# klukaszek/MRI-RayTracer

Hardware: AMD Instinct MI355X
Metric: live Msamples/s, 512^3 fp32 volume @ 1024^2 x 512 steps (gradient shading + ERT) (higher is better)
Workload: dtype f32

## Files before the change

include/mrirt.h:

```cpp
#ifndef MRIRT_H
#define MRIRT_H

#include <stdint.h>

#ifdef __cplusplus
extern "C" {
#endif

#define MRIRT_ABI_VERSION 4

typedef enum MrirtStatus {
    MRIRT_OK = 0,
    MRIRT_ERR_NULL = -1,
    MRIRT_ERR_DIMS = -2,
    MRIRT_ERR_LAYOUT = -3,
    MRIRT_ERR_LAUNCH = -4,
    MRIRT_ERR_ARG = -5,
    MRIRT_ERR_NO_DEVICE = -6
} MrirtStatus;


typedef struct MrirtBratsParams {
    uint32_t imageSize[2]; float fovY; float pad0;
    float eye[3]; float pad1;
// ... 135 lines not shown
int mrirt_build_macro_labels(const uint32_t* labels_linear, const uint32_t dims[3], uint32_t* macro_any, void* stream);
int mrirt_render_brats_skip(const MrirtBratsParams* params, const MrirtRenderExt* ext,
                            const void* const vol[4], const void* labels, const void* preds,
                            const MrirtSkip* skip, void* out_rgba, int64_t pitch_px,
                            uint64_t* stats_dev, void* stream);
int mrirt_brats_skip_applicable(const MrirtBratsParams* params, const MrirtRenderExt* ext, const void* const vol[4],
                                const void* labels, const void* preds, const MrirtSkip* skip);
typedef enum MrirtKernelFamily {
    MRIRT_KERNEL_NONE = 0, MRIRT_KERNEL_GENERIC = 1, MRIRT_KERNEL_PIPELINED = 2, MRIRT_KERNEL_ROLLING = 3,
    MRIRT_KERNEL_SLAB = 4, MRIRT_KERNEL_RING = 5,
    MRIRT_KERNEL_SKIPPING = 16, MRIRT_KERNEL_LABEL_CELLS = 32
} MrirtKernelFamily;
int mrirt_brats_kernel_family(const MrirtBratsParams* params, const MrirtRenderExt* ext, const void* const vol[4],
                              const void* labels, const void* preds, const MrirtSkip* skip);

int64_t mrirt_tiles_for_rank(uint32_t width, uint32_t height, uint32_t tileSize, uint32_t rank, uint32_t world);
int mrirt_detile(const void* gathered, void* frame, uint32_t width, uint32_t height, int64_t pitch_px,
                 uint32_t tileSize, uint32_t world, uint32_t tileSkew, uint32_t outFormat, void* stream);

typedef enum MrirtInrKind {
    MRIRT_INR_FOURIER_RELU = 0,
    MRIRT_INR_SIREN = 1,
    MRIRT_INR_RAW_RELU = 2,
    MRIRT_INR_RAW_SIREN = 3
} MrirtInrKind;

typedef struct MrirtInrDesc {
    uint32_t kind;
    uint32_t numLayers;
    uint32_t inDim;
// ... 184 lines not shown
```

mri-raytracer_amd/_lib.py:

```python
from __future__ import annotations

import ctypes as C
import os
import pathlib
import subprocess
import sys
from typing import List, Optional

PKG_DIR = pathlib.Path(__file__).resolve().parent
CSRC = PKG_DIR / "csrc"
INCLUDE = PKG_DIR.parent / "include"
SO_PATH = pathlib.Path(os.environ.get("MRIRT_LIB", PKG_DIR / "libmrirt.so"))
HIP_SOURCES = ["brats_march.hip", "brats_skip.hip", "brats_c5.hip", "brats_slab.hip", "brats_ring.hip", "brats_backward.hip", "brats_soft.hip", "volume_march.hip", "grid_ops.hip", "inr_mlp.hip",
               "inr_stream.hip", "inr_ws.hip", "inr_refine.hip", "inr_train.hip", "inr_optim.hip", "inr_muon.hip", "inr_lossx.hip", "mesh_rt.hip", "edt.hip", "surface.hip", "abort_trace.cpp"]
HIPCC_FLAGS = ["-O3", "--offload-arch=gfx950", "-ffp-contract=off", "-fPIC", "-shared", "-std=c++17", "-Wall"]

ABI_SYMBOLS = [
    "mrirt_render_brats", "mrirt_render_brats_ex", "mrirt_brats_sample_counts", "mrirt_brats_emit_samples",
    "mrirt_render_brats_stream", "mrirt_brats_inr_scratch_bytes", "mrirt_render_brats_inr", "mrirt_brick_elems", "mrirt_brick_grid",
    "mrirt_unbrick_grid", "mrirt_vec4_elems", "mrirt_vga_elems", "mrirt_build_vec4_grid", "mrirt_build_label_cells", "mrirt_build_mod4_grid", "mrirt_bc4_decode", "mrirt_macro_cells", "mrirt_skip_mask_words",
    "mrirt_build_macro_max", "mrirt_build_macro_labels", "mrirt_render_brats_skip", "mrirt_render_volume", "mrirt_build_cell8", "mrirt_render_sdf", "mrirt_render_mesh", "mrirt_tiles_for_rank",
    "mrirt_detile", "mrirt_inr_pack_bytes", "mrirt_inr_pack_weights", "mrirt_inr_calibrate", "mrirt_inr_forward", "mrirt_inr_forward_refined",
    "mrirt_inr_predict_volume", "mrirt_abi_version", "mrirt_status_string", "mrirt_last_hip_error",
    "mrirt_sizeof", "mrirt_brats_skip_applicable", "mrirt_brats_kernel_family", "mrirt_install_abort_trace",
    "mrirt_edt_scratch_bytes", "mrirt_edt_squared", "mrirt_hausdorff",
    "mrirt_surface_scratch_bytes", "mrirt_surface_count", "mrirt_surface_extract",
    "mrirt_render_brats_backward", "mrirt_render_brats_soft", "mrirt_render_brats_soft_backward",
    "mrirt_inr_train_scratch_bytes", "mrirt_inr_loss_scratch_bytes", "mrirt_inr_forward_f32", "mrirt_inr_loss", "mrirt_inr_backward",
    "mrirt_inr_sample_batch", "mrirt_inr_adamw_scratch_bytes", "mrirt_inr_adamw_step", "mrirt_inr_lr_schedule",
    "mrirt_inr_train_run_scratch_bytes", "mrirt_inr_train_run",
    "mrirt_siren_train_scratch_bytes", "mrirt_siren_forward_f32", "mrirt_siren_backward",
    "mrirt_siren_train_run_scratch_bytes", "mrirt_siren_train_run",
    "mrirt_muon_scratch_bytes", "mrirt_muon_orthogonalize", "mrirt_muon_step",
    "mrirt_inr_train_run_muon_scratch_bytes", "mrirt_inr_train_run_muon",
    "mrirt_inr_loss_ext_scratch_bytes", "mrirt_inr_loss_ext", "mrirt_inr_tumour_count", "mrirt_inr_tumour_index_scratch_bytes",
    "mrirt_inr_tumour_index", "mrirt_inr_sample_batch_mix", "mrirt_inr_train_run_ext_scratch_bytes", "mrirt_inr_train_run_ext",
]

ABI_VERSION = 4
OK = 0
LAYOUT_LINEAR, LAYOUT_BRICK, LAYOUT_VG, LAYOUT_QUAD, LAYOUT_VGA, LAYOUT_LABCELL, LAYOUT_MOD4 = 0, 1, 2, 3, 4, 5, 6
MATH_STRICT, MATH_FAST = 0, 1
OUT_RGBA32F, OUT_RGBA16F = 0, 1
VOX_U32X4, VOX_U8, VOX_F32, VOX_CELL8 = 0, 1, 2, 3
INR_FOURIER_RELU, INR_SIREN = 0, 1
INR_NO_WEIGHT_STATIONARY, INR_NO_REFINE, INR_MARK_ONLY = 1, 2, 4
KERNEL_NONE, KERNEL_GENERIC, KERNEL_PIPELINED, KERNEL_ROLLING, KERNEL_SLAB, KERNEL_RING = 0, 1, 2, 3, 4, 5
KERNEL_SKIPPING, KERNEL_LABEL_CELLS = 16, 32

f32, u32 = C.c_float, C.c_uint32

# ... 89 lines not shown
                ("edemaFpWeight", f32), ("tverskyAlpha", f32), ("tverskyBeta", f32), ("tverskyWeight", f32), ("edemaLogitReg", f32),
                ("edemaClass", u32), ("flags", u32)]


class InrTumourIndex(C.Structure):
    _fields_ = [("index", C.c_void_p), ("offsets", C.c_void_p)]


class InrTrainExt(C.Structure):
    _fields_ = [("loss", C.POINTER(InrLossExt)), ("muon", C.POINTER(Muon)), ("tumour", InrTumourIndex), ("nTumour", C.c_int64)]


class Skip(C.Structure):
    _fields_ = [("macroUb", C.c_void_p * 4), ("macroSeg", C.c_void_p), ("macroPred", C.c_void_p), ("mask", C.c_void_p),
                ("maskWords", u32), ("mapReady", u32)]


class MrirtError(RuntimeError):
    def __init__(self, status: int, where: str):
        l = lib()
        msg = l.mrirt_status_string(status).decode()
        extra = f" (hipError {l.mrirt_last_hip_error()})" if status == -4 else ""
        super().__init__(f"{where}: {msg}{extra} [status {status}]")
        self.status = status


OBJ_DIR = PKG_DIR / "build"
MAX_BUILD_JOBS = 16


# ... 131 lines not shown
    l.mrirt_build_mod4_grid.restype = i32
    l.mrirt_macro_cells.argtypes = [C.POINTER(u32)]
    l.mrirt_macro_cells.restype = i64
    l.mrirt_skip_mask_words.argtypes = [C.POINTER(u32)]
    l.mrirt_skip_mask_words.restype = i64
    l.mrirt_build_macro_max.argtypes = [vp, C.POINTER(u32), vp, vp]
    l.mrirt_build_macro_max.restype = i32
    l.mrirt_build_macro_labels.argtypes = [vp, C.POINTER(u32), vp, vp]
    l.mrirt_build_macro_labels.restype = i32
    l.mrirt_render_brats_skip.argtypes = [C.POINTER(BratsParams), C.POINTER(RenderExt), C.POINTER(vp), vp, vp, C.POINTER(Skip), vp, i64, vp, vp]
    l.mrirt_render_brats_skip.restype = i32
    l.mrirt_brats_skip_applicable.argtypes = [C.POINTER(BratsParams), C.POINTER(RenderExt), C.POINTER(vp), vp, vp, C.POINTER(Skip)]
    l.mrirt_brats_skip_applicable.restype = i32
    l.mrirt_brats_kernel_family.argtypes = l.mrirt_brats_skip_applicable.argtypes
    l.mrirt_brats_kernel_family.restype = i32
    l.mrirt_install_abort_trace.argtypes = [i32]
    l.mrirt_install_abort_trace.restype = i32
    l.mrirt_build_cell8.argtypes = [vp, u32, C.POINTER(u32), vp, vp]
    l.mrirt_build_cell8.restype = i32
    l.mrirt_bc4_decode.argtypes = [vp, u32, u32, u32, vp, vp]
    l.mrirt_bc4_decode.restype = i32
    l.mrirt_render_volume.argtypes = [C.POINTER(VolumeParams), C.POINTER(RenderExt), vp, u32, vp, i64, vp, vp]
    l.mrirt_render_sdf.argtypes = [C.POINTER(SdfParams), u32, u32, vp, i64, vp]
    l.mrirt_render_mesh.argtypes = [C.POINTER(MeshParams), C.POINTER(RenderExt), vp, u32, vp, u32, vp, u32, u32, vp, i64, vp, vp, vp]
    l.mrirt_render_mesh.restype = i32
    l.mrirt_tiles_for_rank.argtypes = [u32, u32, u32, u32, u32]
    l.mrirt_tiles_for_rank.restype = i64
    l.mrirt_detile.argtypes = [vp, vp, u32, u32, i64, u32, u32, u32, u32, vp]
    l.mrirt_inr_pack_bytes.argtypes = [C.POINTER(InrDesc)]
    l.mrirt_inr_pack_bytes.restype = i64
# ... 102 lines not shown
```

mri-raytracer_amd/csrc/brats_device.h:

```cpp
#pragma once
#include "mrirt_host.h"

namespace mrirt {

constexpr uint32_t kMaxStepsPerRay = 1u << 20;

struct K1Args {
    Camera cam;
    PixelMap map;
    GridDims grid;
    VgaDims vga;
    LabelAddr lab;
    float bmin[3], bmax[3];
    UDiv vox[3];
    UDiv wsum;
    UDiv wwDiv;
    float halfInvVoxel[3];
    float hiLin[3];
    float hiLab[3];
    float stepSize, nearT, farT;
    float bg[3];
    uint32_t enabled[4];
    float weight[4];
    float tfLo;
// ... 414 lines not shown
    const bool hit = tmax >= fmaxf(tmin, 0.0f);
    t0 = fmaxf(tmin, fmaxf(0.0f, a.nearT));
    t1 = fminf(tmax, a.farT > 0.0f ? a.farT : tmax);
    return hit && !(t1 <= t0);
}

__device__ __forceinline__ void finish(const K1Args& a, int kind, int64_t oidx, const RayState& r) {
    if (kind != 0) {
        if (a.half) store_rgba<true>(a.out, oidx, r.C0, r.C1, r.C2, 1.0f);
        else        store_rgba<false>(a.out, oidx, r.C0, r.C1, r.C2, 1.0f);
    }
    if (a.stats != nullptr) {
        wave_count_add(a.stats + 0, r.nLive);
        wave_count_add(a.stats + 1, r.nShaded);
    }
}

}
```

mri-raytracer_amd/csrc/brats_host.h:

```cpp
#pragma once
#include "brats_device.h"

namespace mrirt {

struct Prepared { uint32_t layout, math; bool shade, pipe, slab, ring, leap, tag; };

int prepare(const MrirtBratsParams* p, const MrirtRenderExt* ext, const void* const vol[4],
            const void* labels, const void* preds, bool needVolumes, int64_t pitch_px,
            K1Args& a, Prepared& cfg);

int launch_skip_prepass(const MrirtBratsParams* p, const MrirtSkip* skip, bool strict, hipStream_t s, K1Args& a);

int launch_slab_march(const K1Args& a, bool strict, bool shade, hipStream_t s);
int launch_ring_march(const K1Args& a, bool strict, bool shade, hipStream_t s);

int inr_forward_dev_n(const MrirtInrDesc* desc, const float* coords, const float* feats, int64_t nMax,
                      const uint32_t* nDev, int16_t* argmax, uint32_t* segTicket, hipStream_t s);

}
```

mri-raytracer_amd/csrc/brats_march.hip:

```cpp
#include <type_traits>
#include "brats_host.h"
#include "skip_map.h"

namespace mrirt {

template <bool STRICT, int LAYOUT, bool SHADE>
__global__ __launch_bounds__(256) void brats_march_kernel(const K1Args a) {
    using Mm = M<STRICT>;
    __shared__ float4 lutShared[16];
    const float4* lutS = stage_lut(a, lutShared);
    uint32_t px, py;
    int64_t oidx;
    const int kind = map_pixel(a.map, px, py, oidx);
    RayState r = { a.bg[0], a.bg[1], a.bg[2], 1.0f, 0u, 0u };
    float ro[3] = { 0.0f, 0.0f, 0.0f }, rd[3] = { 0.0f, 0.0f, 1.0f }, t0 = 0.0f, t1 = 0.0f;
    const bool marches = kind == 1 && setup_ray(a, px, py, ro, rd, t0, t1);
    WaveGrid<LAYOUT> wg;
    if constexpr (LAYOUT == 4) wg.f = a.vga.ax[vga_pick_axis(a, ro, rd, marches)];
    else wg.g = &a.grid;
    if (marches) {
        float t = t0;
        const int64_t streamBase = a.classStream != nullptr ? a.rayOffsets[(int64_t)py * a.map.width + px] : 0;
        while (t < t1 && r.T > a.ert) {
            Cell s;
// ... 503 lines not shown
    switch (pl.layout) {
        case MRIRT_LAYOUT_LINEAR: k = pl.shade ? layout_kernel<STRICT, 0, true>(pl) : layout_kernel<STRICT, 0, false>(pl); break;
        case MRIRT_LAYOUT_BRICK:  k = pl.shade ? layout_kernel<STRICT, 1, true>(pl) : layout_kernel<STRICT, 1, false>(pl); break;
        case MRIRT_LAYOUT_VG:     k = pl.shade ? layout_kernel<STRICT, 2, true>(pl) : layout_kernel<STRICT, 2, false>(pl); break;
        case MRIRT_LAYOUT_QUAD:   k = layout_kernel<STRICT, 3, false>(pl); break;
        case MRIRT_LAYOUT_VGA:    k = pl.shade ? layout_kernel<STRICT, 4, true>(pl) : layout_kernel<STRICT, 4, false>(pl); break;
        case MRIRT_LAYOUT_MOD4:   k = layout_kernel<STRICT, MRIRT_LAYOUT_MOD4, false>(pl); break;
        default: return MRIRT_ERR_LAYOUT;
    }
    const dim3 grid(a.map.chunk * kXcds), block(a.map.blockPx == 8 ? 64 : 256);
    void* args[] = { const_cast<K1Args*>(&a) };
    MRIRT_HIP(hipLaunchKernel(reinterpret_cast<const void*>(k), grid, block, args, 0, s));
    return MRIRT_OK;
}

int prepare(const MrirtBratsParams* p, const MrirtRenderExt* ext, const void* const vol[4],
            const void* labels, const void* preds, bool needVolumes, int64_t pitch_px,
            K1Args& a, Prepared& cfg) {
    if (!p || (needVolumes && !vol)) return MRIRT_ERR_NULL;
    for (int k = 0; k < 3; ++k) if (p->dims[k] < 2) return MRIRT_ERR_DIMS;
    const uint32_t layout = ext ? ext->layout : (uint32_t)MRIRT_LAYOUT_LINEAR;
    const uint32_t labLayout = ext ? ext->labelLayout : (uint32_t)MRIRT_LAYOUT_LINEAR;
    const uint32_t math = ext ? ext->math : (uint32_t)MRIRT_MATH_STRICT;
    const uint32_t fmt = ext ? ext->outFormat : (uint32_t)MRIRT_OUT_RGBA32F;
    const uint32_t variant = ext ? ext->kernelVariant : 0u;
    const bool labCells = labLayout == MRIRT_LAYOUT_LABCELL;
    const bool mod4 = layout == MRIRT_LAYOUT_MOD4;
    if ((layout > MRIRT_LAYOUT_VGA && !mod4) || (labLayout > MRIRT_LAYOUT_BRICK && !labCells) || math > MRIRT_MATH_FAST || fmt > MRIRT_OUT_RGBA16F)
        return MRIRT_ERR_LAYOUT;
    if (labCells && layout != MRIRT_LAYOUT_QUAD && !mod4) return MRIRT_ERR_LAYOUT;
// ... 17 lines not shown
            const double c = (double)p->volMin[k] + 0.5 * ext - (double)p->eye[k];
            diag2 += ext * ext; dist2 += c * c;
        }
        double tMax = sqrt(dist2) + sqrt(diag2);
        if (ext && ext->cameraMode == 1u)
            tMax += fabs((double)ext->orthoHalfHeight) * (1.0 + (double)p->imageSize[0] / fmax(1.0, (double)p->imageSize[1]));
        if (p->farT > 0.0f && isfinite(p->farT)) tMax = fmin(tMax, (double)p->farT);
        const float tFar = (float)tMax;
        if (!isfinite(tFar) || !(tFar + h > tFar)) return MRIRT_ERR_ARG;
        if (sqrt(diag2) / (double)h > (double)kMaxStepsPerRay) return MRIRT_ERR_ARG;
        if (isnan(p->intensityAlpha)) return MRIRT_ERR_ARG;
        if (!(ext && ext->cameraMode == 1u) && !isfinite(p->fovY)) return MRIRT_ERR_ARG;
        for (int k = 0; k < 3; ++k) if (!isfinite(p->U[k]) || !isfinite(p->V[k]) || !isfinite(p->W[k])) return MRIRT_ERR_ARG;
    }
    fill_camera(a.cam, p->eye, p->U, p->V, p->W, p->fovY, p->imageSize[0], p->imageSize[1], ext, false);
    uint64_t blocks16 = (uint64_t)((p->imageSize[0] + 15u) / 16u) * ((p->imageSize[1] + 15u) / 16u);
    if (ext && ext->tileSize != 0 && ext->tileWorld != 0)
        blocks16 = (uint64_t)mrirt_tiles_for_rank(p->imageSize[0], p->imageSize[1], ext->tileSize, ext->tileRank, ext->tileWorld) *
                   ((ext->tileSize + 15u) / 16u) * ((ext->tileSize + 15u) / 16u);
    const bool bigBlocks = ((variant & 2u) != 0u) != (layout == MRIRT_LAYOUT_VGA && (variant & (64u | 2048u)) == 0u && blocks16 >= 4096u);
    const uint32_t bandSel = (variant >> 4) & 3u;
    const uint32_t bandAsked = bandSel == 0 ? (bigBlocks ? 16u : 8u) : bandSel == 1 ? 16u : bandSel == 2 ? 32u : 64u;
    const uint32_t bandPx = (variant & 8u) ? 0u : bandAsked;
    int rc = fill_pixel_map(a.map, p->imageSize[0], p->imageSize[1], pitch_px, ext,
                            bigBlocks ? 16u : 8u, (variant & 1u) ? 0u : 1u, bandPx,
                            ((variant & 512u) == 0u) != bigBlocks);
    if (rc != MRIRT_OK) return rc;
    fill_grid_dims(a.grid, p->dims, (layout == MRIRT_LAYOUT_VGA || mod4) ? (uint32_t)MRIRT_LAYOUT_VG : layout);
    fill_vga_dims(a.vga, p->dims);
    fill_label_addr(a.lab, p->dims, labCells ? (uint32_t)MRIRT_LAYOUT_LINEAR : labLayout);
    for (int k = 0; k < 3; ++k) {
        a.bmin[k] = p->volMin[k];
        a.bmax[k] = p->volMin[k] + p->voxelSize[k] * (float)p->dims[k];
        a.vox[k] = make_udiv(p->voxelSize[k]);
        a.halfInvVoxel[k] = 0.5f / p->voxelSize[k];
        a.hiLin[k] = (float)p->dims[k] - 1.001f;
        a.hiLab[k] = (float)p->dims[k] - 1.0f;
        a.bg[k] = p->bgColor[k];
    }
    a.stepSize = p->stepSize; a.nearT = p->nearT; a.farT = p->farT;
    float wSum = 0.0f;
// ... 110 lines not shown
}

static int plan_render(const MrirtBratsParams* p, const MrirtRenderExt* ext, const void* const vol[4], const void* labels,
                       const void* preds, const MrirtSkip* skip, int64_t pitch_px, K1Args& a, K1Plan& pl) {
    Prepared cfg;
    const int rc = prepare(p, ext, vol, labels, preds, true, pitch_px, a, cfg);
    if (rc != MRIRT_OK) return rc;
    if (p->showPred != 0 && !preds && a.labCell == nullptr) return MRIRT_ERR_NULL;
    const SkipOffer offer = skip == nullptr ? SkipOffer::None
                          : skip_sound(p, a, skip) && skip->mask != nullptr ? SkipOffer::Map : SkipOffer::NoMap;
    pl = plan_k1(a, cfg, offer);
    if (pl.skipping && (int64_t)skip->maskWords < mrirt_skip_mask_words(p->dims)) return MRIRT_ERR_ARG;
    return pl.status;
}

extern "C" int mrirt_render_brats_skip(const MrirtBratsParams* p, const MrirtRenderExt* ext,
                                       const void* const vol[4], const void* labels, const void* preds,
                                       const MrirtSkip* skip, void* out_rgba, int64_t pitch_px,
                                       uint64_t* stats_dev, void* stream) {
    if (!out_rgba) return MRIRT_ERR_NULL;
    K1Args a;
    K1Plan pl;
    const int rc = plan_render(p, ext, vol, labels, preds, skip, pitch_px, a, pl);
    if (rc != MRIRT_OK) return rc;
    a.out = out_rgba;
    a.stats = stats_dev;
    hipStream_t s = static_cast<hipStream_t>(stream);
    if (pl.skipping) {
        const int rcMap = launch_skip_prepass(p, skip, pl.strict, s, a);
        if (rcMap != MRIRT_OK) return rcMap;
        a.leap = pl.leap ? 1u : 0u;
    }
    return pl.strict ? launch_plan<true>(pl, a, s) : launch_plan<false>(pl, a, s);
}

extern "C" int mrirt_render_brats_ex(const MrirtBratsParams* p, const MrirtRenderExt* ext,
                                     const void* const vol[4], const void* labels, const void* preds,
                                     void* out_rgba, int64_t pitch_px, uint64_t* stats_dev, void* stream) {
    return mrirt_render_brats_skip(p, ext, vol, labels, preds, nullptr, out_rgba, pitch_px, stats_dev, stream);
}

extern "C" int mrirt_brats_skip_applicable(const MrirtBratsParams* p, const MrirtRenderExt* ext, const void* const vol[4],
                                           const void* labels, const void* preds, const MrirtSkip* skip) {
    if (!skip) return 0;
    K1Args a;
    Prepared cfg;
    const int rc = prepare(p, ext, vol, labels, preds, true, p ? (int64_t)p->imageSize[0] : 0, a, cfg);
    if (rc != MRIRT_OK) return rc;
// ... 40 lines not shown
```

mri-raytracer_amd/csrc/mrirt_device.h:

```cpp
#pragma once
#include <hip/hip_runtime.h>
#include <stdint.h>

namespace mrirt {

constexpr int kWave = 64;
constexpr int kTilePx = 8;
constexpr int kBlockPx = 16;
constexpr int kXcds = 8;

#define MRIRT_HD __host__ __device__ __forceinline__
MRIRT_HD uint32_t mul24(uint32_t a, uint32_t b) {
#if defined(__HIP_DEVICE_COMPILE__)
    return __umul24(a, b);
#else
    return a * b;
#endif
}

template <bool STRICT> struct M;

struct UDiv { float d, r; uint32_t exact; };

struct ExpConsts { double log2e, ln2hi, ln2lo, c[13]; };
// ... 223 lines not shown
               ((z >> sh[2]) * mul[2] + (z & mask[2]) * inner[2]);
    }
};

struct PixelMap {
    uint32_t width, height;
    uint32_t blocksX, numBlocks;
    uint32_t chunk;
    uint32_t tileSize, tileRank, tileWorld, tilesX;
    uint32_t tileSkew;
    uint32_t laneOrder;
    uint32_t blockPx;
    uint32_t bandBlocks;
    uint32_t bandShift;
    int64_t  pitch;
};

MRIRT_HD void tile_position(uint32_t t, uint32_t tilesX, uint32_t skew, uint32_t& tx, uint32_t& ty) {
    ty = t / tilesX;
    tx = (t % tilesX + (skew * ty) % tilesX) % tilesX;
}
MRIRT_HD uint32_t tile_dealt_index(uint32_t tx, uint32_t ty, uint32_t tilesX, uint32_t skew) {
    return ty * tilesX + (tx + tilesX - (skew * ty) % tilesX) % tilesX;
}

MRIRT_HD int map_pixel_at(const PixelMap& m, uint32_t b, uint32_t tid, uint32_t& px, uint32_t& py, int64_t& outIndex) {
    uint32_t logical;
    if (m.bandBlocks != 0) {
        const uint32_t xcd = b % kXcds, k = b / kXcds;
        const uint32_t j = k / m.bandBlocks, band = j * kXcds + xcd;
        uint32_t p = k % m.bandBlocks;
        if (m.bandShift != 0) { const uint32_t row = p / m.blocksX, x = (p % m.blocksX + j * m.bandShift) % m.blocksX; p = row * m.blocksX + x; }
        logical = band * m.bandBlocks + p;
    } else {
        logical = (b % kXcds) * m.chunk + b / kXcds;
    }
    if (logical >= m.numBlocks) return 0;
    uint32_t wave = tid >> 6, lane = tid & 63u;
    uint32_t lx, ly;
    if (m.laneOrder == 0) {
        lx = lane & 7u; ly = lane >> 3;
    } else {
        lx = (lane & 1u) | ((lane >> 1) & 2u) | ((lane >> 2) & 4u);
        ly = ((lane >> 1) & 1u) | ((lane >> 2) & 2u) | ((lane >> 3) & 4u);
    }
    lx += (wave & 1u) << 3; ly += (wave >> 1) << 3;
    if (m.tileSize == 0) {
        uint32_t bx = logical % m.blocksX, by = logical / m.blocksX;
        px = bx * m.blockPx + lx; py = by * m.blockPx + ly;
        outIndex = (int64_t)py * m.pitch + px;
    } else {
        uint32_t bpr = m.tileSize / m.blockPx, bpt = bpr * bpr;
        uint32_t lt = logical / bpt, sb = logical % bpt;
        uint32_t t = m.tileRank + lt * m.tileWorld;
        uint32_t tx, ty;
        tile_position(t, m.tilesX, m.tileSkew, tx, ty);
        uint32_t ix = (sb % bpr) * m.blockPx + lx, iy = (sb / bpr) * m.blockPx + ly;
        px = tx * m.tileSize + ix; py = ty * m.tileSize + iy;
        outIndex = ((int64_t)lt * m.tileSize + iy) * m.tileSize + ix;
        return (px < m.width && py < m.height) ? 1 : 2;
    }
    return (px < m.width && py < m.height) ? 1 : 0;
}
__device__ __forceinline__ int map_pixel(const PixelMap& m, uint32_t& px, uint32_t& py, int64_t& outIndex) {
    return map_pixel_at(m, blockIdx.x, threadIdx.x, px, py, outIndex);
}

template <bool HALF>
__device__ __forceinline__ void store_rgba(void* out, int64_t idx, float r, float g, float b, float a) {
    if constexpr (HALF) {
        typedef _Float16 h4 __attribute__((ext_vector_type(4)));
        h4 v = { (_Float16)r, (_Float16)g, (_Float16)b, (_Float16)a };
        reinterpret_cast<h4*>(out)[idx] = v;
    } else {
        reinterpret_cast<float4*>(out)[idx] = make_float4(r, g, b, a);
    }
}

__device__ __forceinline__ void wave_count_add(uint64_t* counter, uint32_t v) {
#pragma unroll
// ... 6 lines not shown
```

mri-raytracer_amd/csrc/mrirt_host.h:

```cpp
#pragma once
#include <hip/hip_runtime.h>
#include <math.h>
#include <stdint.h>
#include <stdlib.h>
#include <string.h>

#include "../../include/mrirt.h"
#include "mrirt_device.h"

namespace mrirt {

extern thread_local int g_last_hip_error;

inline int hip_fail(hipError_t e) {
    g_last_hip_error = (int)e;
    return MRIRT_ERR_LAUNCH;
}

#define MRIRT_HIP(expr)                                         \
    do {                                                        \
        hipError_t e_ = (expr);                                 \
        if (e_ != hipSuccess) return ::mrirt::hip_fail(e_);     \
    } while (0)

// ... 34 lines not shown
    float th = tan_half_fov(fovY);
    c.tanHalf = th;
    c.invTanHalf = 1.0f / th;
    float dimx = (float)width, dimy = (float)height;
    c.aspect = k3Aspect ? dimx / dimy : dimx / fmaxf(1.0f, dimy);
    c.mode = ext ? ext->cameraMode : 0u;
    c.orthoHalfHeight = ext ? ext->orthoHalfHeight : 0.0f;
    c.width = width;
    c.height = height;
}

inline int fill_pixel_map(PixelMap& m, uint32_t width, uint32_t height, int64_t pitch, const MrirtRenderExt* ext,
                          uint32_t blockPx = kBlockPx, uint32_t laneOrder = 0, uint32_t bandPx = 0, bool shiftBands = false) {
    if (width == 0 || height == 0) return MRIRT_ERR_DIMS;
    m.width = width; m.height = height; m.pitch = pitch;
    m.tileSize = ext ? ext->tileSize : 0u;
    m.tileRank = ext ? ext->tileRank : 0u;
    m.tileWorld = ext ? ext->tileWorld : 0u;
    m.tileSkew = 0u;
    m.laneOrder = laneOrder;
    m.blockPx = blockPx;
    if (m.tileSize == 0) {
        if (pitch < (int64_t)width) return MRIRT_ERR_ARG;
        m.tilesX = 0;
        m.blocksX = (width + blockPx - 1) / blockPx;
        m.numBlocks = m.blocksX * ((height + blockPx - 1) / blockPx);
    } else {
        if (m.tileSize % kBlockPx != 0 || m.tileWorld == 0 || m.tileRank >= m.tileWorld) return MRIRT_ERR_ARG;
        if (width > (1u << 20) || height > (1u << 20)) return MRIRT_ERR_DIMS;
        m.tilesX = (width + m.tileSize - 1) / m.tileSize;
// ... 111 lines not shown
```

mri-raytracer_amd/render.py:

```python
from __future__ import annotations

import collections
import contextlib
import ctypes as C
from dataclasses import dataclass
from typing import Any, Dict, Mapping, Optional, Sequence, Tuple, Union

import numpy as np
import torch

from . import _lib
from .params import brats_params, render_ext, sdf_params, volume_params

ArrayLike = Union[np.ndarray, torch.Tensor]


TRACE_HOOK = None


def _require_gpu() -> torch.device:
    if not torch.cuda.is_available():
        raise RuntimeError("mrirt: no HIP device visible — the ray-marcher has no CPU fallback "
                           "(the CPU restatement under oracle/ is test infrastructure only)")
    return torch.device("cuda", torch.cuda.current_device())
# ... 233 lines not shown
        if pred_stream:
            raise ValueError("label cells carry the prediction grid: not with a class stream")
        if P.showPred != 0 and (lab is None or lab.numel() < need[lab_lay]):
            raise ValueError("showPred is set but the label-cell grid is missing or too small")
        prd = None
    elif P.showPred != 0 and not pred_stream and (prd is None or prd.numel() < need[lab_lay]):
        raise ValueError("showPred is set but gPreds is missing or too small")
    return P, E, vols, lab, prd, intensities


KERNEL_FAMILIES = {0: "none", 1: "generic", 2: "pipelined", 3: "rolling", 4: "slab", 5: "ring"}


def kernel_family(params: Mapping[str, Any], ext: Optional[Mapping[str, Any]] = None, skip: bool = False) -> Dict[str, Any]:
    P = brats_params(params)
    E = render_ext(dict(ext or {}))
    fake = C.c_void_p(0x1000)
    vp = (C.c_void_p * 4)(*[fake if (P.volEnabled[m] != 0 or int(E.layout) == _lib.LAYOUT_MOD4) else None for m in range(4)])
    S = None
    if skip:
        S = _lib.Skip()
        for m in range(4):
            S.macroUb[m] = 0x1000 if P.volEnabled[m] != 0 else None
        S.macroSeg = S.macroPred = S.mask = 0x1000
        S.maskWords = 0xFFFFFFFF
    rc = int(_lib.lib().mrirt_brats_kernel_family(C.byref(P), C.byref(E), vp, fake, fake, C.byref(S) if S is not None else None))
    if rc < 0:
        _lib.check(rc, "mrirt_brats_kernel_family")
    return {"family": KERNEL_FAMILIES[rc & 15], "skipping": bool(rc & _lib.KERNEL_SKIPPING), "label_cells": bool(rc & _lib.KERNEL_LABEL_CELLS)}


# ... 59 lines not shown
            entry.empty_fraction = float(_POPCOUNT.to(dev)[bits.long()].sum().item()) / max(cells, 1)
        if entry.empty_fraction < SKIP_MIN_EMPTY_FRACTION:
            return None, None, None
    else:
        if entry is None:
            entry = _SKIP_MAPS[key] = _SkipMap(torch.empty(words, dtype=torch.int32, device=dev), hold, ts)
            while len(_SKIP_MAPS) > _SKIP_MAPS_MAX:
                _SKIP_MAPS.popitem(last=False)
        skip_map_builds += 1
    S.mask, S.maskWords = entry.mask.data_ptr(), words
    hold.append(entry.mask)
    _last_skip_mask = entry.mask
    return S, entry, hold


def render_brats(params: Mapping[str, Any], intensities: Sequence[Optional[Union[ArrayLike, Grid]]],
                 labels: Optional[Union[ArrayLike, Grid]] = None, preds: Optional[Union[ArrayLike, Grid]] = None,
                 out: Optional[torch.Tensor] = None, ext: Optional[Mapping[str, Any]] = None,
                 stats: bool = False, stream=None, skip: bool = False):
    dev = _require_gpu()
    with _on_stream(stream):
        P, E, vols, lab, prd, intensities = _bind_brats(params, intensities, labels, preds, ext, dev)
        o, pitch = _alloc_out(int(P.imageSize[0]), int(P.imageSize[1]), E, dev, out)
        vp = (C.c_void_p * 4)(*[C.c_void_p(t.data_ptr()) if t is not None else None for t in vols])
        st = torch.zeros(2, dtype=torch.int64, device=dev) if stats else None
        if TRACE_HOOK is not None:
            TRACE_HOOK(("[render_brats] " + " ".join(f"{k}={t.data_ptr():#x}+{t.numel() * t.element_size():#x}" for k, t in
                         [(f"vol{m}", v) for m, v in enumerate(vols) if v is not None] + [("lab", lab), ("prd", prd), ("out", o), ("st", st)]
                         if t is not None) + f" skip={skip}\n"))
        S = entry = hold = None
        if skip:
            S, entry, hold = _bind_skip(P, E, vp, lab, prd, intensities, labels, preds, dev, stream)
        if S is not None:
            rc = _lib.lib().mrirt_render_brats_skip(C.byref(P), C.byref(E), vp, _ptr(lab), _ptr(prd), C.byref(S), _ptr(o),
                                                    pitch, _ptr(st), _stream_ptr(stream))
            _lib.check(rc, "mrirt_render_brats_skip")
            entry.built = True
        else:
            rc = _lib.lib().mrirt_render_brats_ex(C.byref(P), C.byref(E), vp, _ptr(lab), _ptr(prd), _ptr(o),
                                                  pitch, _ptr(st), _stream_ptr(stream))
            _lib.check(rc, "mrirt_render_brats_ex")
        if stats:
            s = st.cpu()
            return o, {"live_samples": int(s[0]), "shaded_samples": int(s[1])}
        del hold
    return o


_VOX = {"u32x4": (_lib.VOX_U32X4, torch.int32), "u8": (_lib.VOX_U8, torch.uint8), "f32": (_lib.VOX_F32, torch.float32),
        "cell8": (_lib.VOX_CELL8, torch.int64)}


def build_cell8(volume: ArrayLike, dims: Sequence[int], mode: str = "u8", stream=None) -> torch.Tensor:
    dev = _require_gpu()
    code, dt = _VOX[mode]
    if mode not in ("u8", "u32x4"):
        raise ValueError("build_cell8 takes u8 or u32x4 voxels")
    t = torch.as_tensor(volume)
    if mode == "u32x4" and t.dtype in (torch.uint32, torch.int64):
        t = t.to(torch.int64).to(torch.int32)
# ... 62 lines not shown
```

Before: 157,600.

## Reorder block launch by previous frame's per-block live step counts

Adds a per-block workload record: each wave atomically maxes its live step count into a steps table. Every few frames a small kernel bins blocks into classes by quantile within each XCD and writes a permutation, so later frames launch the heaviest blocks first. The goal is less tail imbalance across CUs and XCDs from uneven ray lengths. The cost is an extra indirection load per block, atomics in the march epilogue, and a periodic sorting kernel. It also uses a workload profile carried over from earlier frames.

```diff
diff --git a/include/mrirt.h b/include/mrirt.h
--- a/include/mrirt.h
+++ b/include/mrirt.h
@@ -173,6 +173,21 @@
 int mrirt_brats_kernel_family(const MrirtBratsParams* params, const MrirtRenderExt* ext, const void* const vol[4],
                               const void* labels, const void* preds, const MrirtSkip* skip);
 
+typedef struct MrirtOrder {
+    uint32_t* order;
+    uint32_t* steps;
+    uint32_t words;
+    uint32_t classes;
+} MrirtOrder;
+int64_t mrirt_order_words(const uint32_t imageSize[2], const MrirtRenderExt* ext);
+int mrirt_render_brats_ordered(const MrirtBratsParams* params, const MrirtRenderExt* ext,
+                               const void* const vol[4], const void* labels, const void* preds,
+                               const MrirtSkip* skip, const MrirtOrder* order, void* out_rgba, int64_t pitch_px,
+                               uint64_t* stats_dev, void* stream);
+int mrirt_brats_order_applicable(const MrirtBratsParams* params, const MrirtRenderExt* ext, const void* const vol[4],
+                                 const void* labels, const void* preds, const MrirtSkip* skip);
+int mrirt_order_build_host(const uint32_t* steps, uint32_t words, uint32_t classes, uint32_t* order);
+
 int64_t mrirt_tiles_for_rank(uint32_t width, uint32_t height, uint32_t tileSize, uint32_t rank, uint32_t world);
 int mrirt_detile(const void* gathered, void* frame, uint32_t width, uint32_t height, int64_t pitch_px,
                  uint32_t tileSize, uint32_t world, uint32_t tileSkew, uint32_t outFormat, void* stream);
diff --git a/mri-raytracer_amd/_lib.py b/mri-raytracer_amd/_lib.py
--- a/mri-raytracer_amd/_lib.py
+++ b/mri-raytracer_amd/_lib.py
@@ -11,7 +11,7 @@
 CSRC = PKG_DIR / "csrc"
 INCLUDE = PKG_DIR.parent / "include"
 SO_PATH = pathlib.Path(os.environ.get("MRIRT_LIB", PKG_DIR / "libmrirt.so"))
-HIP_SOURCES = ["brats_march.hip", "brats_skip.hip", "brats_c5.hip", "brats_slab.hip", "brats_ring.hip", "brats_backward.hip", "brats_soft.hip", "volume_march.hip", "grid_ops.hip", "inr_mlp.hip",
+HIP_SOURCES = ["brats_march.hip", "brats_order.hip", "brats_skip.hip", "brats_c5.hip", "brats_slab.hip", "brats_ring.hip", "brats_backward.hip", "brats_soft.hip", "volume_march.hip", "grid_ops.hip", "inr_mlp.hip",
                "inr_stream.hip", "inr_ws.hip", "inr_refine.hip", "inr_train.hip", "inr_optim.hip", "inr_muon.hip", "inr_lossx.hip", "mesh_rt.hip", "edt.hip", "surface.hip", "abort_trace.cpp"]
 HIPCC_FLAGS = ["-O3", "--offload-arch=gfx950", "-ffp-contract=off", "-fPIC", "-shared", "-std=c++17", "-Wall"]
 
@@ -35,6 +35,7 @@
     "mrirt_inr_train_run_muon_scratch_bytes", "mrirt_inr_train_run_muon",
     "mrirt_inr_loss_ext_scratch_bytes", "mrirt_inr_loss_ext", "mrirt_inr_tumour_count", "mrirt_inr_tumour_index_scratch_bytes",
     "mrirt_inr_tumour_index", "mrirt_inr_sample_batch_mix", "mrirt_inr_train_run_ext_scratch_bytes", "mrirt_inr_train_run_ext",
+    "mrirt_order_words", "mrirt_render_brats_ordered", "mrirt_brats_order_applicable", "mrirt_order_build_host",
 ]
 
 ABI_VERSION = 4
@@ -154,6 +155,10 @@
 class Skip(C.Structure):
     _fields_ = [("macroUb", C.c_void_p * 4), ("macroSeg", C.c_void_p), ("macroPred", C.c_void_p), ("mask", C.c_void_p),
                 ("maskWords", u32), ("mapReady", u32)]
+
+
+class Order(C.Structure):
+    _fields_ = [("order", C.c_void_p), ("steps", C.c_void_p), ("words", u32), ("classes", u32)]
 
 
 class MrirtError(RuntimeError):
@@ -315,6 +320,15 @@
     l.mrirt_brats_skip_applicable.restype = i32
     l.mrirt_brats_kernel_family.argtypes = l.mrirt_brats_skip_applicable.argtypes
     l.mrirt_brats_kernel_family.restype = i32
+    l.mrirt_order_words.argtypes = [C.POINTER(u32), C.POINTER(RenderExt)]
+    l.mrirt_order_words.restype = i64
+    l.mrirt_render_brats_ordered.argtypes = [C.POINTER(BratsParams), C.POINTER(RenderExt), C.POINTER(vp), vp, vp, C.POINTER(Skip), C.POINTER(Order),
+                                             vp, i64, vp, vp]
+    l.mrirt_render_brats_ordered.restype = i32
+    l.mrirt_brats_order_applicable.argtypes = l.mrirt_brats_skip_applicable.argtypes
+    l.mrirt_brats_order_applicable.restype = i32
+    l.mrirt_order_build_host.argtypes = [vp, u32, u32, vp]
+    l.mrirt_order_build_host.restype = i32
     l.mrirt_install_abort_trace.argtypes = [i32]
     l.mrirt_install_abort_trace.restype = i32
     l.mrirt_build_cell8.argtypes = [vp, u32, C.POINTER(u32), vp, vp]
diff --git a/mri-raytracer_amd/csrc/brats_device.h b/mri-raytracer_amd/csrc/brats_device.h
--- a/mri-raytracer_amd/csrc/brats_device.h
+++ b/mri-raytracer_amd/csrc/brats_device.h
@@ -452,6 +452,13 @@
         wave_count_add(a.stats + 0, r.nLive);
         wave_count_add(a.stats + 1, r.nShaded);
     }
-}
-
-}
+    if (a.map.steps != nullptr) {
+        uint32_t v = r.nLive;
+#pragma unroll
+        for (int o = 32; o > 0; o >>= 1) v = max(v, (uint32_t)__shfl_xor(v, o));
+        const uint32_t pos = map_position(a.map);
+        if ((threadIdx.x & 63u) == 0 && v != 0u && pos < a.map.chunk * kXcds) atomicMax(a.map.steps + pos, v);
+    }
+}
+
+}
diff --git a/mri-raytracer_amd/csrc/brats_host.h b/mri-raytracer_amd/csrc/brats_host.h
--- a/mri-raytracer_amd/csrc/brats_host.h
+++ b/mri-raytracer_amd/csrc/brats_host.h
@@ -11,6 +11,8 @@
 
 int launch_skip_prepass(const MrirtBratsParams* p, const MrirtSkip* skip, bool strict, hipStream_t s, K1Args& a);
 
+__attribute__((weak)) int launch_order_build(const K1Args& a, uint32_t classes, hipStream_t s);
+
 int launch_slab_march(const K1Args& a, bool strict, bool shade, hipStream_t s);
 int launch_ring_march(const K1Args& a, bool strict, bool shade, hipStream_t s);
 
diff --git a/mri-raytracer_amd/csrc/brats_march.hip b/mri-raytracer_amd/csrc/brats_march.hip
--- a/mri-raytracer_amd/csrc/brats_march.hip
+++ b/mri-raytracer_amd/csrc/brats_march.hip
@@ -1,6 +1,7 @@
 #include <type_traits>
 #include "brats_host.h"
 #include "skip_map.h"
+#include "k1_order.h"
 
 namespace mrirt {
 
@@ -541,6 +542,22 @@
     return MRIRT_OK;
 }
 
+static int k1_pixel_map(PixelMap& m, const uint32_t imageSize[2], const MrirtRenderExt* ext, int64_t pitch_px) {
+    const uint32_t layout = ext ? ext->layout : (uint32_t)MRIRT_LAYOUT_LINEAR;
+    const uint32_t variant = ext ? ext->kernelVariant : 0u;
+    uint64_t blocks16 = (uint64_t)((imageSize[0] + 15u) / 16u) * ((imageSize[1] + 15u) / 16u);
+    if (ext && ext->tileSize != 0 && ext->tileWorld != 0)
+        blocks16 = (uint64_t)mrirt_tiles_for_rank(imageSize[0], imageSize[1], ext->tileSize, ext->tileRank, ext->tileWorld) *
+                   ((ext->tileSize + 15u) / 16u) * ((ext->tileSize + 15u) / 16u);
+    const bool bigBlocks = ((variant & 2u) != 0u) != (layout == MRIRT_LAYOUT_VGA && (variant & (64u | 2048u)) == 0u && blocks16 >= 4096u);
+    const uint32_t bandSel = (variant >> 4) & 3u;
+    const uint32_t bandAsked = bandSel == 0 ? (bigBlocks ? 16u : 8u) : bandSel == 1 ? 16u : bandSel == 2 ? 32u : 64u;
+    const uint32_t bandPx = (variant & 8u) ? 0u : bandAsked;
+    return fill_pixel_map(m, imageSize[0], imageSize[1], pitch_px, ext,
+                          bigBlocks ? 16u : 8u, (variant & 1u) ? 0u : 1u, bandPx,
+                          ((variant & 512u) == 0u) != bigBlocks);
+}
+
 int prepare(const MrirtBratsParams* p, const MrirtRenderExt* ext, const void* const vol[4],
             const void* labels, const void* preds, bool needVolumes, int64_t pitch_px,
             K1Args& a, Prepared& cfg) {
@@ -588,17 +605,7 @@
         for (int k = 0; k < 3; ++k) if (!isfinite(p->U[k]) || !isfinite(p->V[k]) || !isfinite(p->W[k])) return MRIRT_ERR_ARG;
     }
     fill_camera(a.cam, p->eye, p->U, p->V, p->W, p->fovY, p->imageSize[0], p->imageSize[1], ext, false);
-    uint64_t blocks16 = (uint64_t)((p->imageSize[0] + 15u) / 16u) * ((p->imageSize[1] + 15u) / 16u);
-    if (ext && ext->tileSize != 0 && ext->tileWorld != 0)
-        blocks16 = (uint64_t)mrirt_tiles_for_rank(p->imageSize[0], p->imageSize[1], ext->tileSize, ext->tileRank, ext->tileWorld) *
-                   ((ext->tileSize + 15u) / 16u) * ((ext->tileSize + 15u) / 16u);
-    const bool bigBlocks = ((variant & 2u) != 0u) != (layout == MRIRT_LAYOUT_VGA && (variant & (64u | 2048u)) == 0u && blocks16 >= 4096u);
-    const uint32_t bandSel = (variant >> 4) & 3u;
-    const uint32_t bandAsked = bandSel == 0 ? (bigBlocks ? 16u : 8u) : bandSel == 1 ? 16u : bandSel == 2 ? 32u : 64u;
-    const uint32_t bandPx = (variant & 8u) ? 0u : bandAsked;
-    int rc = fill_pixel_map(a.map, p->imageSize[0], p->imageSize[1], pitch_px, ext,
-                            bigBlocks ? 16u : 8u, (variant & 1u) ? 0u : 1u, bandPx,
-                            ((variant & 512u) == 0u) != bigBlocks);
+    int rc = k1_pixel_map(a.map, p->imageSize, ext, pitch_px);
     if (rc != MRIRT_OK) return rc;
     fill_grid_dims(a.grid, p->dims, (layout == MRIRT_LAYOUT_VGA || mod4) ? (uint32_t)MRIRT_LAYOUT_VG : layout);
     fill_vga_dims(a.vga, p->dims);
@@ -739,10 +746,14 @@
     return pl.status;
 }
 
-extern "C" int mrirt_render_brats_skip(const MrirtBratsParams* p, const MrirtRenderExt* ext,
-                                       const void* const vol[4], const void* labels, const void* preds,
-                                       const MrirtSkip* skip, void* out_rgba, int64_t pitch_px,
-                                       uint64_t* stats_dev, void* stream) {
+static bool order_applies(const K1Plan& pl, const K1Args& a) {
+    return (pl.family == MRIRT_KERNEL_PIPELINED || pl.family == MRIRT_KERNEL_ROLLING) && !pl.skipping && a.map.tileSize == 0;
+}
+
+extern "C" int mrirt_render_brats_ordered(const MrirtBratsParams* p, const MrirtRenderExt* ext,
+                                          const void* const vol[4], const void* labels, const void* preds,
+                                          const MrirtSkip* skip, const MrirtOrder* order, void* out_rgba, int64_t pitch_px,
+                                          uint64_t* stats_dev, void* stream) {
     if (!out_rgba) return MRIRT_ERR_NULL;
     K1Args a;
     K1Plan pl;
@@ -756,7 +767,41 @@
         if (rcMap != MRIRT_OK) return rcMap;
         a.leap = pl.leap ? 1u : 0u;
     }
+    if (order != nullptr && order_applies(pl, a)) {
+        if (!order->order || !order->steps) return MRIRT_ERR_NULL;
+        if (order->classes > kOrderMaxClasses || (uint64_t)order->words < (uint64_t)a.map.chunk * kXcds) return MRIRT_ERR_ARG;
+        a.map.order = order->order;
+        a.map.steps = order->steps;
+        if (order->classes != 0) {
+            if (launch_order_build == nullptr) return MRIRT_ERR_ARG;
+            const int rcOrder = launch_order_build(a, order->classes, s);
+            if (rcOrder != MRIRT_OK) return rcOrder;
+        }
+    }
     return pl.strict ? launch_plan<true>(pl, a, s) : launch_plan<false>(pl, a, s);
+}
+
+extern "C" int mrirt_render_brats_skip(const MrirtBratsParams* p, const MrirtRenderExt* ext,
+                                       const void* const vol[4], const void* labels, const void* preds,
+                                       const MrirtSkip* skip, void* out_rgba, int64_t pitch_px,
+                                       uint64_t* stats_dev, void* stream) {
+    return mrirt_render_brats_ordered(p, ext, vol, labels, preds, skip, nullptr, out_rgba, pitch_px, stats_dev, stream);
+}
+
+extern "C" int mrirt_brats_order_applicable(const MrirtBratsParams* p, const MrirtRenderExt* ext, const void* const vol[4],
+                                            const void* labels, const void* preds, const MrirtSkip* skip) {
+    K1Args a;
+    K1Plan pl;
+    const int rc = plan_render(p, ext, vol, labels, preds, skip, p ? (int64_t)p->imageSize[0] : 0, a, pl);
+    if (rc != MRIRT_OK) return rc;
+    return order_applies(pl, a) ? 1 : 0;
+}
+
+extern "C" int64_t mrirt_order_words(const uint32_t imageSize[2], const MrirtRenderExt* ext) {
+    PixelMap m;
+    if (!imageSize || (ext && ext->tileSize != 0)) return 0;
+    if (k1_pixel_map(m, imageSize, ext, (int64_t)imageSize[0]) != MRIRT_OK) return 0;
+    return (int64_t)m.chunk * kXcds;
 }
 
 extern "C" int mrirt_render_brats_ex(const MrirtBratsParams* p, const MrirtRenderExt* ext,
diff --git a/mri-raytracer_amd/csrc/brats_order.hip b/mri-raytracer_amd/csrc/brats_order.hip
--- /dev/null
+++ b/mri-raytracer_amd/csrc/brats_order.hip
@@ -0,0 +1,122 @@
+#include "brats_host.h"
+#include "k1_order.h"
+
+namespace mrirt {
+
+static_assert(kOrderXcds == kXcds, "the order table is a permutation inside each XCD's slots");
+
+constexpr uint32_t kOrderThreads = 256, kOrderWaves = kOrderThreads / 64;
+constexpr uint32_t kOrderStaged = 4096;
+
+__global__ __launch_bounds__(kOrderThreads) void order_build_kernel(uint32_t* steps, uint32_t words, uint32_t classes, uint32_t* order) {
+    __shared__ uint32_t staged[kOrderStaged];
+    __shared__ uint32_t below[32][kOrderMaxClasses];
+    __shared__ uint32_t total[kOrderMaxClasses], run[kOrderMaxClasses], thrShared[kOrderMaxClasses];
+    __shared__ uint32_t waveCnt[2][kOrderWaves][kOrderMaxClasses];
+    __shared__ uint32_t maxShared;
+    const uint32_t xcd = blockIdx.x, tid = threadIdx.x, lane = tid & 63u, wave = tid >> 6;
+    const uint32_t n = order_slots(words, xcd), C = order_classes(classes);
+    const bool inLds = n <= kOrderStaged;
+    auto record = [&](uint32_t k) { return steps[k * kXcds + xcd]; };
+    auto value = [&](uint32_t k) { return inLds ? staged[k] : record(k); };
+
+    for (uint32_t i = tid; i < 32u * kOrderMaxClasses; i += kOrderThreads) (&below[0][0])[i] = 0u;
+    if (tid < kOrderMaxClasses) { total[tid] = 0u; run[tid] = 0u; }
+    if (tid == 0) maxShared = 0u;
+    __syncthreads();
+    uint32_t vmax = 0;
+    for (uint32_t k = tid; k < n; k += kOrderThreads) {
+        const uint32_t v = record(k);
+        if (inLds) staged[k] = v;
+        vmax = max(vmax, v);
+    }
+#pragma unroll
+    for (int o = 32; o > 0; o >>= 1) vmax = max(vmax, (uint32_t)__shfl_xor(vmax, o));
+    if (lane == 0 && vmax != 0u) atomicMax(&maxShared, vmax);
+    __syncthreads();
+    const uint32_t maxValue = maxShared;
+    if (maxValue == 0u) {
+        for (uint32_t k = tid; k < n; k += kOrderThreads) order[k * kXcds + xcd] = k * kXcds + xcd;
+        return;
+    }
+
+    uint32_t thr[kOrderMaxClasses];
+#pragma unroll
+    for (uint32_t j = 0; j < kOrderMaxClasses; ++j) thr[j] = 0u;
+    uint32_t trip = 0;
+    for (uint32_t bit = order_top_bit(maxValue); bit != 0u; bit >>= 1, ++trip) {
+        for (uint32_t base = 0; base < n; base += kOrderThreads) {
+            const uint32_t k = base + tid;
+            const bool have = k < n;
+            const uint32_t v = have ? value(k) : 0u;
+#pragma unroll
+            for (uint32_t j = 0; j < kOrderMaxClasses - 1; ++j) {
+                if (j + 1 < C) {
+                    const uint32_t cnt = (uint32_t)__popcll(__ballot(have && v < (thr[j] | bit)));
+                    if (lane == 0 && cnt != 0u) atomicAdd(&below[trip][j], cnt);
+                }
+            }
+        }
+        __syncthreads();
+#pragma unroll
+        for (uint32_t j = 0; j < kOrderMaxClasses - 1; ++j)
+            if (j + 1 < C) thr[j] = order_refine(thr[j], bit, below[trip][j], order_rank(j + 1, n, C));
+    }
+
+    if (tid == 0) {
+#pragma unroll
+        for (uint32_t j = 0; j < kOrderMaxClasses; ++j) thrShared[j] = thr[j];
+    }
+    __syncthreads();
+
+    for (uint32_t base = 0; base < n; base += kOrderThreads) {
+        const uint32_t k = base + tid;
+        const uint32_t c = k < n ? order_class(value(k), thrShared, C) : ~0u;
+        for (uint32_t cc = 0; cc < C; ++cc) {
+            const uint32_t cnt = (uint32_t)__popcll(__ballot(c == cc));
+            if (lane == 0 && cnt != 0u) atomicAdd(&total[cc], cnt);
+        }
+    }
+    __syncthreads();
+    uint32_t it = 0;
+    for (uint32_t base = 0; base < n; base += kOrderThreads, ++it) {
+        const uint32_t k = base + tid, buf = it & 1u;
+        const uint32_t c = k < n ? order_class(value(k), thrShared, C) : ~0u;
+        uint32_t rankInWave = 0;
+        for (uint32_t cc = 0; cc < C; ++cc) {
+            const uint64_t b = __ballot(c == cc);
+            if (c == cc) rankInWave = (uint32_t)__popcll(b & ((1ull << lane) - 1ull));
+            if (lane == 0) waveCnt[buf][wave][cc] = (uint32_t)__popcll(b);
+        }
+        __syncthreads();
+        if (k < n) {
+            uint32_t pos = run[c] + rankInWave;
+            for (uint32_t cc = c + 1; cc < C; ++cc) pos += total[cc];
+            for (uint32_t w = 0; w < wave; ++w) pos += waveCnt[buf][w][c];
+            if (pos < n) order[pos * kXcds + xcd] = k * kXcds + xcd;
+        }
+        __syncthreads();
+        if (tid < C) { uint32_t s = 0; for (uint32_t w = 0; w < kOrderWaves; ++w) s += waveCnt[buf][w][tid]; run[tid] += s; }
+    }
+    __syncthreads();
+    for (uint32_t k = tid; k < n; k += kOrderThreads) steps[k * kXcds + xcd] = 0u;
+}
+
+int launch_order_build(const K1Args& a, uint32_t classes, hipStream_t s) {
+    uint32_t* order = const_cast<uint32_t*>(a.map.order);
+    uint32_t* steps = a.map.steps;
+    uint32_t words = a.map.chunk * kXcds;
+    void* args[] = { &steps, &words, &classes, &order };
+    MRIRT_HIP(hipLaunchKernel(reinterpret_cast<const void*>(order_build_kernel), dim3(kXcds), dim3(kOrderThreads), args, 0, s));
+    return MRIRT_OK;
+}
+
+}
+
+using namespace mrirt;
+
+extern "C" int mrirt_order_build_host(const uint32_t* steps, uint32_t words, uint32_t classes, uint32_t* order) {
+    if (words != 0 && (!steps || !order)) return MRIRT_ERR_NULL;
+    order_build_table(steps, words, classes, order);
+    return MRIRT_OK;
+}
diff --git a/mri-raytracer_amd/csrc/k1_order.h b/mri-raytracer_amd/csrc/k1_order.h
--- /dev/null
+++ b/mri-raytracer_amd/csrc/k1_order.h
@@ -0,0 +1,64 @@
+#pragma once
+#include <stdint.h>
+
+#if defined(__HIPCC__)
+#define MRIRT_ORDER_HD __host__ __device__ inline
+#else
+#define MRIRT_ORDER_HD inline
+#endif
+
+namespace mrirt {
+
+constexpr uint32_t kOrderXcds = 8;
+constexpr uint32_t kOrderMaxClasses = 16;
+constexpr uint32_t kOrderDefaultClasses = 4;
+
+MRIRT_ORDER_HD uint32_t order_classes(uint32_t classes) {
+    return classes == 0 ? kOrderDefaultClasses : classes > kOrderMaxClasses ? kOrderMaxClasses : classes;
+}
+MRIRT_ORDER_HD uint32_t order_slots(uint32_t words, uint32_t xcd) {
+    return xcd < words ? (words - xcd + kOrderXcds - 1) / kOrderXcds : 0u;
+}
+MRIRT_ORDER_HD uint32_t order_rank(uint32_t j, uint32_t n, uint32_t C) { return (uint32_t)(((uint64_t)j * n) / C); }
+MRIRT_ORDER_HD uint32_t order_refine(uint32_t ans, uint32_t bit, uint32_t below, uint32_t k) { return below <= k ? (ans | bit) : ans; }
+MRIRT_ORDER_HD uint32_t order_top_bit(uint32_t maxValue) {
+    uint32_t bit = 1u;
+    while ((maxValue >> 1) >= bit) bit <<= 1;
+    return bit;
+}
+MRIRT_ORDER_HD uint32_t order_class(uint32_t v, const uint32_t* thr, uint32_t C) {
+    uint32_t c = 0;
+    for (uint32_t j = 0; j + 1 < C; ++j) c += v >= thr[j] ? 1u : 0u;
+    return c;
+}
+
+inline void order_build_xcd(const uint32_t* steps, uint32_t words, uint32_t xcd, uint32_t classes, uint32_t* order) {
+    const uint32_t n = order_slots(words, xcd), C = order_classes(classes);
+    uint32_t maxValue = 0;
+    for (uint32_t k = 0; k < n; ++k) { const uint32_t v = steps[k * kOrderXcds + xcd]; maxValue = v > maxValue ? v : maxValue; }
+    if (maxValue == 0) {
+        for (uint32_t k = 0; k < n; ++k) order[k * kOrderXcds + xcd] = k * kOrderXcds + xcd;
+        return;
+    }
+    uint32_t thr[kOrderMaxClasses] = {};
+    for (uint32_t j = 1; j < C; ++j) {
+        const uint32_t rank = order_rank(j, n, C);
+        uint32_t ans = 0;
+        for (uint32_t bit = order_top_bit(maxValue); bit != 0; bit >>= 1) {
+            uint32_t below = 0;
+            for (uint32_t k = 0; k < n; ++k) below += steps[k * kOrderXcds + xcd] < (ans | bit) ? 1u : 0u;
+            ans = order_refine(ans, bit, below, rank);
+        }
+        thr[j - 1] = ans;
+    }
+    uint32_t pos = 0;
+    for (uint32_t c = C; c-- > 0;)
+        for (uint32_t k = 0; k < n; ++k)
+            if (order_class(steps[k * kOrderXcds + xcd], thr, C) == c) order[(pos++) * kOrderXcds + xcd] = k * kOrderXcds + xcd;
+}
+
+inline void order_build_table(const uint32_t* steps, uint32_t words, uint32_t classes, uint32_t* order) {
+    for (uint32_t xcd = 0; xcd < kOrderXcds; ++xcd) order_build_xcd(steps, words, xcd, classes, order);
+}
+
+}
diff --git a/mri-raytracer_amd/csrc/mrirt_device.h b/mri-raytracer_amd/csrc/mrirt_device.h
--- a/mri-raytracer_amd/csrc/mrirt_device.h
+++ b/mri-raytracer_amd/csrc/mrirt_device.h
@@ -261,6 +261,8 @@
     uint32_t bandBlocks;
     uint32_t bandShift;
     int64_t  pitch;
+    const uint32_t* order;
+    uint32_t* steps;
 };
 
 MRIRT_HD void tile_position(uint32_t t, uint32_t tilesX, uint32_t skew, uint32_t& tx, uint32_t& ty) {
@@ -271,7 +273,7 @@
     return ty * tilesX + (tx + tilesX - (skew * ty) % tilesX) % tilesX;
 }
 
-MRIRT_HD int map_pixel_at(const PixelMap& m, uint32_t b, uint32_t tid, uint32_t& px, uint32_t& py, int64_t& outIndex) {
+MRIRT_HD uint32_t map_logical(const PixelMap& m, uint32_t b) {
     uint32_t logical;
     if (m.bandBlocks != 0) {
         const uint32_t xcd = b % kXcds, k = b / kXcds;
@@ -282,6 +284,11 @@
     } else {
         logical = (b % kXcds) * m.chunk + b / kXcds;
     }
+    return logical;
+}
+
+MRIRT_HD int map_pixel_at(const PixelMap& m, uint32_t b, uint32_t tid, uint32_t& px, uint32_t& py, int64_t& outIndex) {
+    const uint32_t logical = map_logical(m, b);
     if (logical >= m.numBlocks) return 0;
     uint32_t wave = tid >> 6, lane = tid & 63u;
     uint32_t lx, ly;
@@ -309,8 +316,11 @@
     }
     return (px < m.width && py < m.height) ? 1 : 0;
 }
+__device__ __forceinline__ uint32_t map_position(const PixelMap& m) {
+    return m.order != nullptr ? m.order[blockIdx.x] : blockIdx.x;
+}
 __device__ __forceinline__ int map_pixel(const PixelMap& m, uint32_t& px, uint32_t& py, int64_t& outIndex) {
-    return map_pixel_at(m, blockIdx.x, threadIdx.x, px, py, outIndex);
+    return map_pixel_at(m, map_position(m), threadIdx.x, px, py, outIndex);
 }
 
 template <bool HALF>
diff --git a/mri-raytracer_amd/csrc/mrirt_host.h b/mri-raytracer_amd/csrc/mrirt_host.h
--- a/mri-raytracer_amd/csrc/mrirt_host.h
+++ b/mri-raytracer_amd/csrc/mrirt_host.h
@@ -72,6 +72,7 @@
                           uint32_t blockPx = kBlockPx, uint32_t laneOrder = 0, uint32_t bandPx = 0, bool shiftBands = false) {
     if (width == 0 || height == 0) return MRIRT_ERR_DIMS;
     m.width = width; m.height = height; m.pitch = pitch;
+    m.order = nullptr; m.steps = nullptr;
     m.tileSize = ext ? ext->tileSize : 0u;
     m.tileRank = ext ? ext->tileRank : 0u;
     m.tileWorld = ext ? ext->tileWorld : 0u;
diff --git a/mri-raytracer_amd/render.py b/mri-raytracer_amd/render.py
--- a/mri-raytracer_amd/render.py
+++ b/mri-raytracer_amd/render.py
@@ -271,7 +271,9 @@
 
 def kernel_family(params: Mapping[str, Any], ext: Optional[Mapping[str, Any]] = None, skip: bool = False) -> Dict[str, Any]:
     P = brats_params(params)
-    E = render_ext(dict(ext or {}))
+    ext = dict(ext or {})
+    ext.pop("order", None)
+    E = render_ext(ext)
     fake = C.c_void_p(0x1000)
     vp = (C.c_void_p * 4)(*[fake if (P.volEnabled[m] != 0 or int(E.layout) == _lib.LAYOUT_MOD4) else None for m in range(4)])
     S = None
@@ -361,11 +363,52 @@
     return S, entry, hold
 
 
+ORDER_DEFAULT = True
+ORDER_CLASSES = 4
+ORDER_REBUILD_EVERY = 8
+ORDER_MAP_BITS = 0xA7B
+_ORDERS: "collections.OrderedDict[tuple, list]" = collections.OrderedDict()
+_ORDERS_MAX = 16
+order_binds = 0
+
+
+def _bind_order(P, E, vp, lab, prd, S, pitch, dev, stream):
+    global order_binds
+    lib = _lib.lib()
+    rc = int(lib.mrirt_brats_order_applicable(C.byref(P), C.byref(E), vp, _ptr(lab), _ptr(prd), C.byref(S) if S is not None else None))
+    if rc < 0:
+        _lib.check(rc, "mrirt_brats_order_applicable")
+    size = (C.c_uint32 * 2)(int(P.imageSize[0]), int(P.imageSize[1]))
+    words = int(lib.mrirt_order_words(size, C.byref(E)))
+    if rc == 0 or words == 0:
+        return None, None
+    ts = _as_stream(stream)
+    key = (dev.index, int(ts.cuda_stream), int(P.imageSize[0]), int(P.imageSize[1]), int(pitch), words, int(E.layout),
+           int(E.kernelVariant) & ORDER_MAP_BITS)
+    entry = _ORDERS.get(key)
+    if entry is None:
+        entry = _ORDERS[key] = [torch.zeros(2 * words, dtype=torch.int32, device=dev), 0]
+        while len(_ORDERS) > _ORDERS_MAX:
+            _ORDERS.popitem(last=False)
+    else:
+        _ORDERS.move_to_end(key)
+    t, frame = entry
+    entry[1] = frame + 1
+    O = _lib.Order()
+    O.order, O.steps = t.data_ptr(), t.data_ptr() + 4 * words
+    O.words = words
+    O.classes = ORDER_CLASSES if frame < 2 or frame % max(1, ORDER_REBUILD_EVERY) == 0 else 0
+    order_binds += 1
+    return O, t
+
+
 def render_brats(params: Mapping[str, Any], intensities: Sequence[Optional[Union[ArrayLike, Grid]]],
                  labels: Optional[Union[ArrayLike, Grid]] = None, preds: Optional[Union[ArrayLike, Grid]] = None,
                  out: Optional[torch.Tensor] = None, ext: Optional[Mapping[str, Any]] = None,
                  stats: bool = False, stream=None, skip: bool = False):
     dev = _require_gpu()
+    ext = dict(ext or {})
+    ordered = bool(ext.pop("order", ORDER_DEFAULT))
     with _on_stream(stream):
         P, E, vols, lab, prd, intensities = _bind_brats(params, intensities, labels, preds, ext, dev)
         o, pitch = _alloc_out(int(P.imageSize[0]), int(P.imageSize[1]), E, dev, out)
@@ -378,7 +421,16 @@
         S = entry = hold = None
         if skip:
             S, entry, hold = _bind_skip(P, E, vp, lab, prd, intensities, labels, preds, dev, stream)
-        if S is not None:
+        O = otab = None
+        if ordered:
+            O, otab = _bind_order(P, E, vp, lab, prd, S, pitch, dev, stream)
+        if O is not None:
+            rc = _lib.lib().mrirt_render_brats_ordered(C.byref(P), C.byref(E), vp, _ptr(lab), _ptr(prd), C.byref(S) if S is not None else None,
+                                                       C.byref(O), _ptr(o), pitch, _ptr(st), _stream_ptr(stream))
+            _lib.check(rc, "mrirt_render_brats_ordered")
+            if entry is not None:
+                entry.built = True
+        elif S is not None:
             rc = _lib.lib().mrirt_render_brats_skip(C.byref(P), C.byref(E), vp, _ptr(lab), _ptr(prd), C.byref(S), _ptr(o),
                                                     pitch, _ptr(st), _stream_ptr(stream))
             _lib.check(rc, "mrirt_render_brats_skip")
@@ -390,7 +442,7 @@
         if stats:
             s = st.cpu()
             return o, {"live_samples": int(s[0]), "shaded_samples": int(s[1])}
-        del hold
+        del hold, otab
     return o
 
 
```

Result: faster. 160,500 (median of 6 runs) (+1.8%).
